# DiamondLightSource/fast-feedback-service

Measured on AMD Instinct MI355X. Metric: detector frames/s (Eiger-16M 4362x4148 uint16), higher is better.
Workload: dtype u16; 1 GPU; eiger16m: 4148x4362 uint16, 7x7 dispersion window, 32 frames/step/GPU resident in HBM, spots+centroids returned to host; streams=4, parallelism=single GPU, spot_gather=none (single GPU)

## Files before the change

fast-feedback-service_amd/csrc/ffs_context.hip:

```cpp
#include <sys/mman.h>

#include "ffs_internal.hpp"
#include "kernels_mask.hpp"

static_assert(sizeof(ReflOut) == sizeof(ffs_reflection), "record layout");
static_assert(offsetof(ReflOut, sum_intensity) == offsetof(ffs_reflection, sum_intensity), "record layout");

thread_local std::string g_create_error;

static void ctx_destroy_internal(ffs_ctx* c);
namespace {
struct Registry {
    std::mutex mu;
    std::unordered_set<const void*> live[3];
    std::atomic<bool> exiting{false};
    bool exit_hook_installed = false;
};
Registry& registry() {
    static Registry* r = new Registry();
    return *r;
}
static void on_process_exit() {
    Registry& r = registry();
    std::vector<ffs_ctx*> ctxs;
// ... 248 lines not shown
    }
    for (ffs_stream* s : streams)
        if (handle_take(kHandleStream, s)) stream_destroy_internal(s);
    for (ffs_stack3d* st : stacks)
        if (handle_take(kHandleStack, st)) {
            g_live_stacks.fetch_sub(1);
            stack3d_free(st);
        }
    ctx_destroy_internal(c);
}

static void ctx_destroy_internal(ffs_ctx* c) {
    (void)hipSetDevice(c->device);
    ahead_stop(c, true);
    for (auto* st : c->stack_pool) stack3d_free(st);
    c->stack_pool.clear();
    if (AssemblyPool* pool = c->assembly.exchange(nullptr)) {
        pool->owner.lock();
        pool->owner.unlock();
        delete pool;
    }
    if (c->d_maskbits) (void)hipFree(c->d_maskbits);
    if (c->d_gain_map) (void)hipFree(c->d_gain_map);
    if (c->d_radial_map) (void)hipFree(c->d_radial_map);
    if (c->stats_st) {
        (void)hipStreamSynchronize(c->stats_st);
        (void)hipStreamDestroy(c->stats_st);
    }
    if (c->d_stats) (void)hipFree(c->d_stats);
    if (c->d_ginfo) (void)hipFree(c->d_ginfo);
    if (c->d_mmap) (void)hipFree(c->d_mmap);
    if (c->dense_st) (void)hipStreamDestroy(c->dense_st);
    if (c->dense_st2) (void)hipStreamDestroy(c->dense_st2);
    if (c->d_handoff) (void)hipFree(c->d_handoff);
    if (c->up_st) (void)hipStreamDestroy(c->up_st);
    for (auto st : c->sparse_st) if (st) (void)hipStreamDestroy(st);
    for (auto e : c->chain_ev) if (e) (void)hipEventDestroy(e);
    for (auto& pb : c->pinned_pool) pinned_free(pb);
    delete c;
}

static int rebuild_mask_tables(ffs_ctx* c) {
    const Layout& L = c->L;
    const uint32_t gpitch = ginfo_pitch(L, c->pixel_bytes);
    HIP_TRY(c, hipMemset(c->d_ginfo, 0, (size_t)(L.H + kInfoExtraRows) * gpitch));
    const int groups = L.pitch_px / (c->pixel_bytes == 2 ? 8 : 4);
    (void)hipGetLastError();
    if (c->pixel_bytes == 2)
        hipLaunchKernelGGL(k_build_maps, dim3((groups + 255) / 256, L.H), dim3(256), 0, 0, c->d_maskbits, L.mpitch, L.W, L.H,
                           L.pitch_px, c->d_mmap, c->d_ginfo, gpitch);
    else
        hipLaunchKernelGGL(k_build_maps4, dim3((groups + 255) / 256, L.H), dim3(256), 0, 0, c->d_maskbits, L.mpitch, L.W, L.H,
                           L.pitch_px, c->d_mmap, c->d_ginfo, gpitch);
    HIP_TRY(c, hipGetLastError());
    c->empty_runs = EmptyRuns{};
    uint8_t* d_flags = nullptr;
    HIP_TRY(c, hipMalloc(reinterpret_cast<void**>(&d_flags), (size_t)L.H));
    hipLaunchKernelGGL(k_row_flags, dim3((unsigned)L.H), dim3(64), 0, 0, c->d_maskbits, L.mpitch, L.H, d_flags);
    std::vector<uint8_t> flags((size_t)L.H, 1);
    hipError_t e = hipGetLastError();
    if (e == hipSuccess) e = hipMemcpy(flags.data(), d_flags, flags.size(), hipMemcpyDeviceToHost);
    (void)hipFree(d_flags);
    HIP_TRY(c, e);
    HIP_TRY(c, hipDeviceSynchronize());
    c->empty_runs = empty_runs_of(flags.data(), L.H);
    return FFS_OK;
}

static int ffs_ctx_set_mask_impl(ffs_ctx* c, const uint8_t* host_mask) {
    if (!c) return FFS_ERR_INVALID;
    const Layout& L = c->L;
    std::vector<uint8_t> bits(L.plane_frame_stride, 0);
    const int full = L.W / 8;
    for (int y = 0; y < L.H; ++y) {
        uint8_t* row = bits.data() + (size_t)y * L.mpitch;
        if (host_mask) {
            const uint8_t* m = host_mask + (size_t)y * L.W;
            for (int g = 0; g < full; ++g) {
                uint64_t v;
                std::memcpy(&v, m + 8 * g, 8);
                const uint64_t nz = (((v & 0x7F7F7F7F7F7F7F7Full) + 0x7F7F7F7F7F7F7F7Full) | v) & 0x8080808080808080ull;
                row[g] = (uint8_t)(((nz >> 7) * 0x0102040810204080ull) >> 56);
            }
            for (int x = full * 8; x < L.W; ++x)
                if (m[x]) row[x >> 3] |= (uint8_t)(1u << (x & 7));
        } else {
            std::memset(row, 0xFF, (size_t)full);
            for (int x = full * 8; x < L.W; ++x) row[x >> 3] |= (uint8_t)(1u << (x & 7));
        }
    }
    HIP_TRY(c, hipSetDevice(c->device));
    HIP_TRY(c, hipMemcpy(c->d_maskbits, bits.data(), bits.size(), hipMemcpyHostToDevice));
    return rebuild_mask_tables(c);
}

static int ffs_ctx_get_mask_impl(ffs_ctx* c, uint8_t* host_mask) {
    if (!c || !host_mask) return FFS_ERR_INVALID;
    const Layout& L = c->L;
    std::vector<uint8_t> bits(L.plane_frame_stride);
    HIP_TRY(c, hipSetDevice(c->device));
    HIP_TRY(c, hipMemcpy(bits.data(), c->d_maskbits, bits.size(), hipMemcpyDeviceToHost));
    for (int y = 0; y < L.H; ++y)
        for (int x = 0; x < L.W; ++x)
            host_mask[(size_t)y * L.W + x] = (bits[(size_t)y * L.mpitch + (x >> 3)] >> (x & 7)) & 1;
    return FFS_OK;
}
// ... 493 lines not shown
```

fast-feedback-service_amd/csrc/kernels_mask.hpp:

```cpp
#pragma once
#include "ffs_device.h"

namespace ffsamd {

__global__ __launch_bounds__(256) void k_build_maps(const uint8_t* maskbits, uint32_t mpitch, int W, int H, int pitch_px,
                                                    uint8_t* mmap, uint8_t* ginfo, uint32_t gpitch_bytes) {
    const int g = blockIdx.x * 256 + threadIdx.x;
    const int y = blockIdx.y;
    if (g * 8 >= pitch_px) return;
    uint32_t cnt[8] = {0, 0, 0, 0, 0, 0, 0, 0};
    for (int dy = -3; dy <= 3; ++dy) {
        const int yy = y + dy;
        if (yy < 0 || yy >= H) continue;
        const uint8_t* row = maskbits + (uint64_t)yy * mpitch;
        uint32_t b = (uint32_t)row[g] << 8;
        if (g > 0) b |= row[g - 1];
        if ((uint32_t)(g + 1) < mpitch) b |= (uint32_t)row[g + 1] << 16;
        for (int j = 0; j < 8; ++j) cnt[j] += __popc((b >> (j + 5)) & 0x7Fu);
    }
    const uint32_t own = maskbits[(uint64_t)y * mpitch + g];
    uint32_t mn = 255, mx = 0;
    for (int j = 0; j < 8; ++j) {
        mmap[(uint64_t)y * pitch_px + g * 8 + j] = (uint8_t)cnt[j];
        if ((own >> j) & 1u) { mn = min(mn, cnt[j]); mx = max(mx, cnt[j]); }
    }
    if (mx == 0) mn = 0;
    ginfo[(uint64_t)y * gpitch_bytes + g * 4] = (uint8_t)own;
    ginfo[(uint64_t)(y + kInfoExtraRows) * gpitch_bytes + g * 4 + 1] = (uint8_t)mn;
    ginfo[(uint64_t)(y + kInfoExtraRows) * gpitch_bytes + g * 4 + 2] = (uint8_t)mx;
    ginfo[(uint64_t)(y + kInfoExtraRows) * gpitch_bytes + g * 4 + 3] = (uint8_t)own;
}

__global__ __launch_bounds__(256) void k_build_maps4(const uint8_t* maskbits, uint32_t mpitch, int W, int H, int pitch_px,
                                                     uint8_t* mmap, uint8_t* ginfo, uint32_t gpitch_bytes) {
    const int g = blockIdx.x * 256 + threadIdx.x;
    const int y = blockIdx.y;
    if (g * 4 >= pitch_px) return;
    uint32_t cnt[4] = {0, 0, 0, 0};
    const int byte0 = (g * 4) >> 3, sh = (g * 4) & 7;
    for (int dy = -3; dy <= 3; ++dy) {
        const int yy = y + dy;
        if (yy < 0 || yy >= H) continue;
        const uint8_t* row = maskbits + (uint64_t)yy * mpitch;
        uint32_t b = (uint32_t)row[byte0] << 8;
        if (byte0 > 0) b |= row[byte0 - 1];
        if ((uint32_t)(byte0 + 1) < mpitch) b |= (uint32_t)row[byte0 + 1] << 16;
        for (int j = 0; j < 4; ++j) cnt[j] += __popc((b >> (5 + sh + j)) & 0x7Fu);
    }
    const uint32_t own = (maskbits[(uint64_t)y * mpitch + byte0] >> sh) & 0xFu;
    uint32_t mn = 255, mx = 0;
    for (int j = 0; j < 4; ++j) {
        mmap[(uint64_t)y * pitch_px + g * 4 + j] = (uint8_t)cnt[j];
        if ((own >> j) & 1u) { mn = min(mn, cnt[j]); mx = max(mx, cnt[j]); }
    }
    if (mx == 0) mn = 0;
    ginfo[(uint64_t)y * gpitch_bytes + g * 4] = (uint8_t)own;
    ginfo[(uint64_t)(y + kInfoExtraRows) * gpitch_bytes + g * 4 + 1] = (uint8_t)mn;
    ginfo[(uint64_t)(y + kInfoExtraRows) * gpitch_bytes + g * 4 + 2] = (uint8_t)mx;
    ginfo[(uint64_t)(y + kInfoExtraRows) * gpitch_bytes + g * 4 + 3] = (uint8_t)own;
}

__global__ __launch_bounds__(64) void k_row_flags(const uint8_t* maskbits, uint32_t mpitch, int H, uint8_t* flags) {
    const int y = blockIdx.x;
    if (y >= H) return;
    const uint32_t* row = reinterpret_cast<const uint32_t*>(maskbits + (uint64_t)y * mpitch);
    uint32_t any = 0;
    for (uint32_t w = threadIdx.x; w < mpitch / 4; w += 64) any |= row[w];
    const unsigned long long m = __ballot(any != 0u);
    if (threadIdx.x == 0) flags[y] = m != 0ull ? 1 : 0;
}

__global__ void k_resolution_mask(uint8_t* maskbits, uint32_t mpitch, int W, int H, float wavelength,
                                  float distance, float cx, float cy, float psx, float psy,
                                  float dmin, float dmax) {
    const int bx = blockIdx.x * blockDim.x + threadIdx.x;
    const int y = blockIdx.y;
    if (bx * 8 >= W || y >= H) return;
    uint8_t* p = maskbits + (uint64_t)y * mpitch + bx;
    uint32_t b = *p;
    for (int j = 0; j < 8; ++j) {
        const int x = bx * 8 + j;
        if (x >= W || !((b >> j) & 1u)) continue;
        const float dx = (((float)x + 0.5f) - cx) * psx;
        const float dy = (((float)y + 0.5f) - cy) * psy;
        const float r = sqrtf(dx * dx + dy * dy);
        const float theta = 0.5f * atanf(r / distance);
        const float res = wavelength / (2.0f * sinf(theta));
        if ((dmin > 0 && res < dmin) || (dmax > 0 && res > dmax)) b &= ~(1u << j);
    }
    *p = (uint8_t)b;
}

}
```

fast-feedback-service_amd/csrc/kernels_stream.hpp:

```cpp
#pragma once
#include "kernels_threshold.hpp"

#ifndef FFS_IMG_LOAD_AUX
#define FFS_IMG_LOAD_AUX 0
#endif

namespace ffsamd {

constexpr int kSQWords = 32;

__device__ __forceinline__ bool exact_predicate(const ThresholdArgs& a, uint32_t m, unsigned long long sx,
                                                unsigned long long sy, uint32_t pc) {
    const double src = (double)pc;
    if (!((int)m >= a.min_count && src > a.threshold)) return false;
    if (a.max_valid >= 0 && (long long)pc > a.max_valid) return false;
    const double md = (double)m, xd = (double)sx, yd = (double)sy;
    const double t0 = md * yd;
    const double t1 = xd * xd;
    const double t2 = xd * (md - 1.0);
    const double av = (t0 - t1) - t2;
    const double bv = md * src - xd;
    const double cv = (xd * a.nsig_b) * __builtin_sqrt(2.0 * (md - 1.0));
    const double dv = a.nsig_s * __builtin_sqrt(xd * md);
    return av > cv && bv > dv;
// ... 71 lines not shown
__global__ __launch_bounds__(64, 4) void k_stream_u16(const ThresholdArgs a) {
    __shared__ uint32_t s_q[kSQWords][kQCap];
    __shared__ uint16_t s_list[kQCap * 8];

    const int lane = threadIdx.x;
    if (a.dbg_prio & 1) __builtin_amdgcn_s_setprio(3);
    int strip, band;
    const bool real = stream_unit(a, blockIdx.x, strip, band);
    if constexpr (!EXT)
        if (a.handoff && blockIdx.x == gridDim.x - 1 && blockIdx.y == gridDim.y - 1 && lane == 0)
            __hip_atomic_store(a.handoff, a.handoff_seq, __ATOMIC_RELEASE, __HIP_MEMORY_SCOPE_SYSTEM);
    if (!real) return;
    [[maybe_unused]] const uint32_t slot = log_slot(a, blockIdx.y, (uint32_t)band, (uint32_t)strip);
    const int f0 = blockIdx.y * a.group_frames;
    const int nf = min(a.group_frames, a.n_frames - f0);
    const int band0 = band_first_row(band, a.band_rows, a.band_rows2, a.band_split);
    const int band1 = min(band_first_row(band + 1, a.band_rows, a.band_rows2, a.band_split), a.H);
    const BandRows rows = DENSE ? BandRows{band0, band1} : trim_band(a.empty_runs, band0, band1);
    const int yb0 = rows.yb0, yb1 = rows.yb1;

    const int gsep = a.gpf + 1;
    const int G = strip * kSOwned + lane - 1;
    const int fl = G >= 0 ? G / gsep : 0;
    const int g = G - fl * gsep;
    const bool active = G >= 0 && fl < nf && g < a.gpf && yb0 != yb1;
    const bool owned = active && lane >= 1 && lane <= kSOwned;
    const uint32_t my_fg = ((uint32_t)fl << 16) | (uint32_t)g;

    const rsrc_t r_img = make_rsrc((const uint8_t*)a.image + (uint64_t)f0 * a.frame_stride,
                                   (uint32_t)((uint64_t)(nf - 1) * a.frame_stride + (uint64_t)a.H * a.pitch));
    const rsrc_t r_info = make_rsrc(a.ginfo, (uint32_t)(a.H + kInfoExtraRows) * a.gpitch);
    const rsrc_t r_sb = make_rsrc(a.strong_bytes + (uint64_t)f0 * a.bytes_frame_stride,
                                  (uint32_t)((uint64_t)nf * a.bytes_frame_stride));
    const rsrc_t r_cb = make_rsrc((EXT ? a.dplane : a.bits) + (uint64_t)f0 * a.plane_frame_stride, (uint32_t)((uint64_t)nf * a.plane_frame_stride));
    constexpr uint32_t kOob = 0x80000000u;
    const uint32_t off_px = active ? (uint32_t)((uint64_t)fl * a.frame_stride) + (uint32_t)g * 16u : kOob;
    const uint32_t off_info = active ? (uint32_t)g * 4u : kOob;
    uint32_t off_byte_st;
    {
        const uint32_t lpf = a.bpitch >> 7;
        const uint32_t u = (uint32_t)strip * 4u + ((uint32_t)lane >> 4);
        const uint32_t fz = u / lpf, cz = u - fz * lpf;
        off_byte_st = fz < (uint32_t)nf ? (uint32_t)((uint64_t)fz * a.bytes_frame_stride) + cz * 128u + ((uint32_t)lane & 15u) * 8u : kOob;
    }

    const int total = (yb1 - yb0) + (FFS_DBG(a, 1024) ? 0 : 6);
    const float kS = a.kS;

    constexpr int NS = 7 + KAHEAD;
    uint32_t ring[NS][4];
    uint32_t rinfo[NS];
    uint32_t col[8], colq[8];
    uint32_t M[4] = {0, 0, 0, 0};
    uint32_t mprev = 0;
    typedef float f32x2 __attribute__((ext_vector_type(2)));
    [[maybe_unused]] f32x2 ext_c1 = {0.0f, 0.0f}, ext_c2 = {0.0f, 0.0f};
#pragma unroll
    for (int s = 0; s < NS; ++s) {
        rinfo[s] = 0;
#pragma unroll
        for (int q = 0; q < 4; ++q) ring[s][q] = 0;
    }
#pragma unroll
    for (int j = 0; j < 8; ++j) { col[j] = 0; colq[j] = 0; }
    const unsigned long long owned_mask = __builtin_amdgcn_ballot_w64(owned);

    auto fetch = [&](int slot, int i) {
        const int yin = yb0 - 3 + i;
        const uint32_t prow = (uint32_t)min(max(yin, 0), a.H - 1);
        const uint32_t irow = (uint32_t)min(max(yin, 0), a.H + kInfoExtraRows - 1);
        const u32x4 v = __builtin_amdgcn_raw_buffer_load_b128(r_img, off_px, prow * a.pitch, FFS_IMG_LOAD_AUX);
        ring[slot][0] = v[0]; ring[slot][1] = v[1]; ring[slot][2] = v[2]; ring[slot][3] = v[3];
        rinfo[slot] = __builtin_amdgcn_raw_buffer_load_b32(r_info, off_info | (yin < 0 ? kOob : 0u), (FFS_DBG(a, 64) ? 8u : irow) * a.gpitch, 0);
    };

    auto mask_row = [&](int slot, int slot_before) {
        if (__ballot(rinfo[slot] != rinfo[slot_before]) != 0ull) {
            const uint32_t mb = rinfo[slot] & 0xFFu;
            if (__ballot(mb != mprev) != 0ull) {
#pragma unroll
                for (int q = 0; q < 4; ++q)
                    M[q] = ((uint32_t)__builtin_amdgcn_sbfe((int)mb, 2 * q, 1) & 0xFFFFu)
                         | ((uint32_t)__builtin_amdgcn_sbfe((int)mb, 2 * q + 1, 1) & 0xFFFF0000u);
                mprev = mb;
            }
            if constexpr (EXT) {
                const uint32_t mmin = (rinfo[slot] >> 8) & 0xFFu, mmax = (rinfo[slot] >> 16) & 0xFFu;
                const float mm1 = (float)mmin - 1.0f;
                const float c1 = (float)mmax * 1.0000019073486328125f;
                const float c2 = (mm1 + a.kB * __builtin_amdgcn_sqrtf(2.0f * mm1)) * 0.99999952316284179688f;
                ext_c1 = f32x2{c1, c1};
                ext_c2 = f32x2{c2, c2};
            }
        }
#pragma unroll
        for (int q = 0; q < 4; ++q) {
            ring[slot][q] &= M[q];
            asm("" : "+v"(ring[slot][q]));
        }
    };

    auto push = [&](int s, int so) {
#pragma unroll
        for (int q = 0; q < 4; ++q) {
            const uint32_t wn = ring[s][q], wo = ring[so][q];
            {
                const int32_t t = (int32_t)((wn & 0xFFFFu) - (wo & 0xFFFFu));
                const int32_t u = (int32_t)((wn & 0xFFFFu) + (wo & 0xFFFFu));
                col[2 * q] += (uint32_t)t;
                colq[2 * q] += (uint32_t)__mul24(t, u);
            }
            {
                const int32_t t = (int32_t)((wn >> 16) - (wo >> 16));
                const int32_t u = (int32_t)((wn >> 16) + (wo >> 16));
                col[2 * q + 1] += (uint32_t)t;
                colq[2 * q + 1] += (uint32_t)__mul24(t, u);
            }
        }
    };

    int qn = 0;
    [[maybe_unused]] uint32_t nlog = 0;
    [[maybe_unused]] uint32_t nbuf = 0;
    [[maybe_unused]] uint32_t lbuf[6] = {0, 0, 0, 0, 0, 0};
    [[maybe_unused]] auto flush_log = [&]() {
        const uint32_t at = nlog + (uint32_t)lane;
        if ((uint32_t)lane < nbuf && at < (uint32_t)kWlogCap && !FFS_DBG(a, 512)) {
            a.wlog[(uint64_t)slot * kWlogCap + at] = make_uint2(lbuf[0], lbuf[1]);
            a.wpix[(uint64_t)slot * kWlogCap + at] = make_uint4(lbuf[2], lbuf[3], lbuf[4], lbuf[5]);
        }
        nlog += nbuf;
        nbuf = 0;
    };
    auto drain = [&]() {
        const bool have = lane < qn && !FFS_DBG(a, 2) && !FFS_DBG(a, 32);
        uint32_t todo = 0, row = 0, fe = 0, ge = 0;
        if (have) {
            uint32_t xs[8], pws[4];
#pragma unroll
            for (int j = 0; j < 8; ++j) xs[j] = s_q[j][lane];
#pragma unroll
            for (int q = 0; q < 4; ++q) pws[q] = s_q[8 + q][lane];
            row = s_q[30][lane] >> 6;
            const uint32_t fg = s_q[31][lane];
            fe = fg >> 16;
            ge = fg & 0xFFFFu;
            const uint32_t ginf = s_q[15][lane];
            const uint32_t gmin = (ginf >> 8) & 0xFFu, gmax = (ginf >> 16) & 0xFFu;
            uint2 mm = make_uint2(gmin * 0x01010101u, gmin * 0x01010101u);
            if (gmin != gmax) {
                uint2 t = *reinterpret_cast<const uint2*>(a.mmap + (uint64_t)min(row, (uint32_t)a.H - 1u) * a.pitch_px + min(ge * 8u, (uint32_t)a.pitch_px - 8u));
                asm volatile("" : "+v"(t.x), "+v"(t.y));
                mm = t;
            }
            s_q[12][lane] = mm.x;
            s_q[13][lane] = mm.y;
            s_q[14][lane] = 0u;
            uint32_t sure = 0;
            if constexpr (EXT) {
                const uint32_t valid = ginf >> 24;
                const float kq_group = a.kB * __builtin_amdgcn_sqrtf(2.0f * ((float)gmin - 1.0f));
#pragma unroll
                for (int j = 0; j < 8; ++j) {
                    const uint32_t x = xs[j];
                    const uint32_t pw = pws[j >> 1];
                    const uint32_t pv = (j & 1) ? pw >> 16 : pw & 0xFFFFu;
                    const uint32_t m = ((j < 4 ? mm.x : mm.y) >> (8 * (j & 3))) & 0xFFu;
                    const float mf = (float)m, xf = (float)x, yf = (float)s_q[16 + j][lane];
                    const float kq = gmin == gmax ? kq_group : a.kB * __builtin_amdgcn_sqrtf(2.0f * (mf - 1.0f));
                    const float t0 = mf * yf;
                    const float af = t0 - xf * (xf + (mf - 1.0f));
                    const float cf = xf * kq;
                    const float slack = t0 * 9.5367431640625e-07f;
                    const bool bright = x >= 65536u;
                    const bool maybe = (af + slack >= cf) || bright;
                    const bool yes = !bright && (af - slack > cf * 1.000003814697265625f);
                    const bool ok = ((valid >> j) & 1u) && (int)m >= a.min_count && !(a.max_valid >= 0 && (long long)pv > a.max_valid);
                    todo |= (ok && maybe && !yes) ? (1u << j) : 0u;
                    sure |= (ok && yes) ? (1u << j) : 0u;
                }
                s_q[14][lane] = sure;
            } else {
#pragma unroll
                for (int j = 0; j < 8; ++j) {
                    const uint32_t x = xs[j];
                    const uint32_t pw = pws[j >> 1];
                    const uint32_t pv = (j & 1) ? pw >> 16 : pw & 0xFFFFu;
                    const uint32_t m = ((j < 4 ? mm.x : mm.y) >> (8 * (j & 3))) & 0xFFu;
                    const int32_t b = (int32_t)__umul24(m, pv) - (int32_t)x;
                    const float bf = (float)b, tf = (float)__umul24(x, m);
                    todo |= (bf * __builtin_fabsf(bf) > kS * tf) ? (1u << j) : 0u;
                }
            }
            if (FFS_DBG(a, 4)) todo = 0;
        }
        const uint32_t todo_n = (uint32_t)__popc(todo);
        const uint32_t todo_incl = wave_inclusive_scan(todo_n);
        const int T = __builtin_amdgcn_readlane((int)todo_incl, 63);
        {
            uint32_t pos = todo_incl - todo_n, w = todo;
            while (w) {
                const uint32_t j = (uint32_t)__ffs((int)w) - 1u;
                w &= w - 1u;
                s_list[pos++] = (uint16_t)(((uint32_t)lane << 3) | j);
            }
        }
        __builtin_amdgcn_wave_barrier();
        for (int base = 0; base < T; base += 64) {
            const int idx = base + lane;
            if (idx < T) {
                const uint32_t ent = s_list[idx], e = ent >> 3, j = ent & 7u;
                const uint32_t x = s_q[j][e], pv = (s_q[8 + (j >> 1)][e] >> (16 * (j & 1))) & 0xFFFFu;
                const uint32_t m = (s_q[12 + (j >> 2)][e] >> (8 * (j & 3))) & 0xFFu;
                uint32_t y = 0;
                if constexpr (EXT) {
                    y = s_q[16 + j][e];
                } else {
#pragma unroll
                    for (uint32_t t = 0; t < 7; ++t) y += s_q[16 + j + t][e];
                }
                asm volatile("" : "+v"(y));
                if (x < 65536u) {
                    bool certain;
                    bool strong;
                    if constexpr (EXT) {
                        strong = dispersion_only_nosqrt(a, m, x, y, certain);
                        if (!certain) strong = dispersion_only(a, m, x, y);
                    } else {
                        if (a.int_pred) strong = int_predicate(a, m, x, y, pv, certain);
                        else strong = exact_predicate_nosqrt(a, m, x, y, pv, certain);
                        if (!certain) strong = exact_predicate(a, m, x, y, pv);
                    }
                    if (strong) atomicOr(&s_q[14][e], 1u << j);
                } else if (!EXT && a.bright_to_plane) {
                    atomicOr(&s_q[14][e], 1u << j);
                } else if (!EXT && a.wlog) {
                    atomicOr(&s_q[14][e], 0x100u << j);
                } else {
                    const uint32_t tg = s_q[30][e], fgc = s_q[31][e];
                    const uint32_t fc = fgc >> 16, gc = fgc & 0xFFFFu;
                    const uint32_t at = atomicAdd(a.bright_n, 1u);
                    if (at < a.bright_cap)
                        a.bright_list[at] = make_uint2(((uint32_t)(f0 + (int)fc) << 16) | (gc * 8u + j), tg >> 6);
                }
            }
        }
        __builtin_amdgcn_wave_barrier();
        if constexpr (!EXT) if (a.wlog) {
            const uint32_t cbm = have ? s_q[14][lane] : 0u;
            const uint32_t pxw[4] = {s_q[8][lane], s_q[9][lane], s_q[10][lane], s_q[11][lane]};
            const unsigned long long wm = __builtin_amdgcn_ballot_w64(cbm != 0u);
            if (wm) {
                const uint32_t cnt = (uint32_t)__popcll(wm);
                if (nbuf + cnt > 64u) flush_log();
                const uint32_t rank = __builtin_amdgcn_mbcnt_hi((uint32_t)(wm >> 32), __builtin_amdgcn_mbcnt_lo((uint32_t)wm, 0u));
                const uint32_t dump = nbuf + cnt < 64u ? nbuf + cnt : 0u;
                const int to = (int)((cbm != 0u ? nbuf + rank : dump) << 2);
                const uint32_t e0 = (uint32_t)__builtin_amdgcn_ds_permute(to, (int)((row << 16) | ge));
                const uint32_t e1 = (uint32_t)__builtin_amdgcn_ds_permute(to, (int)((fe << 16) | cbm));
                const uint32_t p0 = (uint32_t)__builtin_amdgcn_ds_permute(to, (int)pxw[0]), p1 = (uint32_t)__builtin_amdgcn_ds_permute(to, (int)pxw[1]);
                const uint32_t p2 = (uint32_t)__builtin_amdgcn_ds_permute(to, (int)pxw[2]), p3 = (uint32_t)__builtin_amdgcn_ds_permute(to, (int)pxw[3]);
                if ((uint32_t)lane - nbuf < cnt) {
                    lbuf[0] = e0; lbuf[1] = e1;
                    lbuf[2] = p0; lbuf[3] = p1; lbuf[4] = p2; lbuf[5] = p3;
                }
                nbuf += cnt;
            }
            qn = 0;
            return;
        }
        if (have) {
            const uint32_t cb = s_q[14][lane];
            if (cb) {
                if (!FFS_DBG(a, 256)) __builtin_amdgcn_raw_buffer_store_b8((uint8_t)cb, r_cb, (uint32_t)((uint64_t)fe * a.plane_frame_stride) + ge, row * a.mpitch, 0);
                if constexpr (!EXT) if (!FFS_DBG(a, 128)) {
                    atomicAdd(a.tile_counts + (uint64_t)(f0 + (int)fe) * a.n_tiles + (row / (uint32_t)kTileRows), (uint32_t)__popc(cb));
                    const uint32_t ob = row * a.occ_spr + (ge >> 4);
                    atomicOr(a.occ + (uint64_t)(f0 + (int)fe) * a.occ_frame_words + (ob >> 5), 1u << (ob & 31u));
                }
            }
        }
        qn = 0;
    };

#pragma unroll
    for (int s = 0; s < KAHEAD; ++s) fetch(s, s);

#pragma unroll
    for (int s = 0; s < 6; ++s) {
        mask_row(s, (s + NS - 1) % NS);
        push(s, (s + KAHEAD) % NS);
        fetch((s + KAHEAD) % NS, s + KAHEAD);
    }

    for (int base = 6;; base += NS) {
#pragma unroll
        for (int t = 0; t < NS; ++t) {
            const int s = (6 + t) % NS;
            const int so = (s + KAHEAD) % NS;
            const int sc = (s + NS - 3) % NS;
            const int i = base + t;
            if (i >= total) goto rows_done;
            {
                const uint32_t info = rinfo[s];
                mask_row(s, (s + NS - 1) % NS);
                push(s, so);
                fetch(so, i + KAHEAD);

                const uint32_t s01 = col[0] + col[1], s23 = col[2] + col[3], s45 = col[4] + col[5], s67 = col[6] + col[7];
                const uint32_t ua = s01 + s23, va = s45 + s67;
                const uint32_t T0 = dpp_shr_add(s67, ua);
                const uint32_t T1 = ua + s45;
                const uint32_t T2 = va + s23;
                const uint32_t T3 = dpp_shl_add(s01, va);
                uint32_t Wn[8];
                Wn[0] = dpp_shr_add(col[5], T0);
                Wn[1] = T0 + col[4];
                Wn[2] = dpp_shr_add(col[7], T1);
                Wn[3] = T1 + col[6];
                Wn[4] = T2 + col[1];
                Wn[5] = dpp_shl_add(col[0], T2);
                Wn[6] = T3 + col[3];
                Wn[7] = dpp_shl_add(col[2], T3);

                const int yout = __builtin_amdgcn_readfirstlane(yb0 + (i - 6));
                const uint32_t so_bytes = (uint32_t)yout * a.bpitch;

                const uint32_t xmin = min(min(min(min(Wn[0], Wn[1]), Wn[2]), min(min(Wn[3], Wn[4]), Wn[5])), min(Wn[6], Wn[7]));
                const uint32_t mmin = (info >> 8) & 0xFFu, mmax = (info >> 16) & 0xFFu;
                bool pass;
                [[maybe_unused]] uint32_t ys[8];
                if constexpr (EXT) {
                    const uint32_t q01 = colq[0] + colq[1], q23 = colq[2] + colq[3], q45 = colq[4] + colq[5], q67 = colq[6] + colq[7];
                    const uint32_t qa = q01 + q23, qb = q45 + q67;
                    const uint32_t U0 = dpp_shr_add(q67, qa), U1 = qa + q45, U2 = qb + q23, U3 = dpp_shl_add(q01, qb);
                    const uint32_t y0 = dpp_shr_add(colq[5], U0), y1 = U0 + colq[4], y2 = dpp_shr_add(colq[7], U1), y3 = U1 + colq[6];
                    const uint32_t y4 = U2 + colq[1], y5 = dpp_shl_add(colq[0], U2), y6 = U3 + colq[3], y7 = dpp_shl_add(colq[2], U3);
                    ys[0] = y0; ys[1] = y1; ys[2] = y2; ys[3] = y3; ys[4] = y4; ys[5] = y5; ys[6] = y6; ys[7] = y7;
                    float dmax = -1.0f;
#pragma unroll
                    for (int jp = 0; jp < 4; ++jp) {
                        const f32x2 xf = {(float)Wn[2 * jp], (float)Wn[2 * jp + 1]};
                        const f32x2 yf = {(float)ys[2 * jp], (float)ys[2 * jp + 1]};
                        const f32x2 u = xf * (xf + ext_c2);
                        const f32x2 d = __builtin_elementwise_fma(ext_c1, yf, -u);
                        dmax = __builtin_fmaxf(dmax, __builtin_fmaxf(d.x, d.y));
                    }
                    const uint32_t xmax = max(max(max(max(Wn[0], Wn[1]), Wn[2]), max(max(Wn[3], Wn[4]), Wn[5])), max(Wn[6], Wn[7]));
                    pass = mmax != 0u && (dmax >= 0.0f || xmax >= 65536u);
                } else {
                    uint32_t pmax;
                    {
                        typedef uint16_t u16x2 __attribute__((ext_vector_type(2)));
                        const u16x2 a01 = __builtin_bit_cast(u16x2, ring[sc][0]), a23 = __builtin_bit_cast(u16x2, ring[sc][1]);
                        const u16x2 a45 = __builtin_bit_cast(u16x2, ring[sc][2]), a67 = __builtin_bit_cast(u16x2, ring[sc][3]);
                        const u16x2 mx = __builtin_elementwise_max(__builtin_elementwise_max(a01, a23), __builtin_elementwise_max(a45, a67));
                        const uint32_t mw = __builtin_bit_cast(uint32_t, mx);
                        pmax = max(mw & 0xFFFFu, mw >> 16);
                    }
                    const int32_t B = (int32_t)__umul24(mmax, pmax) - (int32_t)xmin;
                    const float bf = (float)B, tf = (float)__umul24(xmin, mmin);
                    float lhs = bf * __builtin_fabsf(bf);
                    asm("" : "+v"(lhs));
                    pass = lhs > kS * tf;
                }
                if constexpr (DENSE) __builtin_amdgcn_raw_buffer_store_b64(u32x2{0u, 0u}, r_sb, off_byte_st, so_bytes, 2 );
                const unsigned long long fm = FFS_DBG(a, 1) ? 0ull : (__builtin_amdgcn_ballot_w64(pass) & owned_mask);
                const bool flag = pass && owned;
                if (fm) {
                    const int nfl = __popcll(fm);
                    if (qn + nfl > kQCap) drain();
                    if constexpr (EXT) {
                        if (flag && !FFS_DBG(a, 32)) {
                            const uint32_t rank = __builtin_amdgcn_mbcnt_hi((uint32_t)(fm >> 32), __builtin_amdgcn_mbcnt_lo((uint32_t)fm, 0u));
                            const int e = qn + (int)rank;
#pragma unroll
                            for (int w = 0; w < 8; ++w) {
                                s_q[w][e] = Wn[w];
                                s_q[16 + w][e] = ys[w];
                            }
#pragma unroll
                            for (int w = 0; w < 4; ++w) s_q[8 + w][e] = ring[sc][w];
                            s_q[15][e] = info;
                            s_q[30][e] = ((uint32_t)yout << 6) | (uint32_t)lane; s_q[31][e] = my_fg;
                        }
                    } else {
                    const uint32_t QL5 = from_left(colq[5]), QL6 = from_left(colq[6]), QL7 = from_left(colq[7]);
                    const uint32_t QR0 = from_right(colq[0]), QR1 = from_right(colq[1]), QR2 = from_right(colq[2]);
                    if (flag && !FFS_DBG(a, 32)) {
                        const uint32_t rank = __builtin_amdgcn_mbcnt_hi((uint32_t)(fm >> 32), __builtin_amdgcn_mbcnt_lo((uint32_t)fm, 0u));
                        const int e = qn + (int)rank;
#pragma unroll
                        for (int w = 0; w < 8; ++w) {
                            s_q[w][e] = Wn[w];
                            s_q[19 + w][e] = colq[w];
                        }
#pragma unroll
                        for (int w = 0; w < 4; ++w) s_q[8 + w][e] = ring[sc][w];
                        s_q[15][e] = info;
                        s_q[16][e] = QL5; s_q[17][e] = QL6; s_q[18][e] = QL7;
                        s_q[27][e] = QR0; s_q[28][e] = QR1; s_q[29][e] = QR2;
                        s_q[30][e] = ((uint32_t)yout << 6) | (uint32_t)lane; s_q[31][e] = my_fg;
                    }
                    }
                    qn += nfl;
                }
            }
        }
    }
rows_done:
    if (qn > 0) drain();
    if constexpr (!EXT) if (a.wlog) {
        flush_log();
        if (lane == 0) a.wlog_n[slot] = FFS_DBG(a, 512) ? 0u : nlog;
    }
}
template <typename PixelT, bool EXT = false>
__global__ __launch_bounds__(256) void k_bright_fix(const ThresholdArgs a) {
    if (blockIdx.x == 0 && threadIdx.x == 0 && *a.bright_n > a.bright_cap) atomicOr(a.overflow, kOvfBrightList);
    const uint32_t n = min(*a.bright_n, a.bright_cap);
    for (uint32_t e = blockIdx.x * 256 + threadIdx.x; e < n; e += gridDim.x * 256) {
        const uint2 r = a.bright_list[e];
        const uint32_t frame = r.x >> 16, x = r.x & 0xFFFFu, y = r.y;
        const uint8_t* img = (const uint8_t*)a.image + (uint64_t)frame * a.frame_stride;
        if (exact_strong<PixelT, EXT>(a, img, (int)x, (int)y)) {
            uint8_t* plane = (EXT ? a.dplane : a.bits) + (uint64_t)frame * a.plane_frame_stride + (uint64_t)y * a.mpitch;
            atomicOr(reinterpret_cast<uint32_t*>(plane) + (x >> 5), 1u << (x & 31u));
            if (!EXT) {
                atomicAdd(a.tile_counts + (uint64_t)frame * a.n_tiles + y / (uint32_t)kTileRows, 1u);
                const uint32_t ob = y * a.occ_spr + (x >> 7);
                atomicOr(a.occ + (uint64_t)frame * a.occ_frame_words + (ob >> 5), 1u << (ob & 31u));
            }
        }
    }
}


constexpr int kS4Words = 32;

template <int KAHEAD, bool DENSE = false>
__global__ __launch_bounds__(64, 4) void k_stream_u32(const ThresholdArgs a) {
    __shared__ uint32_t s_q[kS4Words][kQCap];
    __shared__ uint16_t s_list[kQCap * 4];

    const int lane = threadIdx.x;
    int strip, band;
    const bool real = stream_unit(a, blockIdx.x, strip, band);
    if (a.handoff && blockIdx.x == gridDim.x - 1 && blockIdx.y == gridDim.y - 1 && lane == 0)
        __hip_atomic_store(a.handoff, a.handoff_seq, __ATOMIC_RELEASE, __HIP_MEMORY_SCOPE_SYSTEM);
    if (!real) return;
    const uint32_t slot = log_slot(a, blockIdx.y, (uint32_t)band, (uint32_t)strip);
    const int f0 = blockIdx.y * a.group_frames;
    const int nf = min(a.group_frames, a.n_frames - f0);
    const int band0 = band_first_row(band, a.band_rows, a.band_rows2, a.band_split);
    const int band1 = min(band_first_row(band + 1, a.band_rows, a.band_rows2, a.band_split), a.H);
    const BandRows rows = DENSE ? BandRows{band0, band1} : trim_band(a.empty_runs, band0, band1);
    const int yb0 = rows.yb0, yb1 = rows.yb1;

    const int gsep = a.gpf + 1;
    const int G = strip * kSOwned + lane - 1;
    const int fl = G >= 0 ? G / gsep : 0;
    const int g = G - fl * gsep;
    const bool active = G >= 0 && fl < nf && g < a.gpf && yb0 != yb1;
    const bool owned = active && lane >= 1 && lane <= kSOwned;

    const rsrc_t r_img = make_rsrc((const uint8_t*)a.image + (uint64_t)f0 * a.frame_stride,
                                   (uint32_t)((uint64_t)(nf - 1) * a.frame_stride + (uint64_t)a.H * a.pitch));
    const rsrc_t r_info = make_rsrc(a.ginfo, (uint32_t)(a.H + kInfoExtraRows) * a.gpitch);
    const rsrc_t r_sb = make_rsrc(a.strong_bytes + (uint64_t)f0 * a.bytes_frame_stride,
                                  (uint32_t)((uint64_t)nf * a.bytes_frame_stride));
    constexpr uint32_t kOob = 0x80000000u;
    const uint32_t off_px = active ? (uint32_t)((uint64_t)fl * a.frame_stride) + (uint32_t)g * 16u : kOob;
    const uint32_t off_info = active ? (uint32_t)g * 4u : kOob;
    uint32_t off_byte_st;
    {
        const uint32_t lpf = a.bpitch >> 7;
        const uint32_t u = (uint32_t)strip * 2u + ((uint32_t)lane >> 4);
        const uint32_t fz = u / lpf, cz = u - fz * lpf;
        off_byte_st = (lane < 32 && fz < (uint32_t)nf) ? (uint32_t)((uint64_t)fz * a.bytes_frame_stride) + cz * 128u + ((uint32_t)lane & 15u) * 8u : kOob;
    }

    const int total = (yb1 - yb0) + 6;
    const float kS = a.kS;

    constexpr int NS = 7 + KAHEAD;
    uint32_t ring[NS][4];
    uint32_t rinfo[NS];
    uint32_t col[4];
    long long colq[4];
    uint32_t M[4] = {0, 0, 0, 0};
    uint32_t mprev = 0;
    uint32_t bighist = 0;
#pragma unroll
    for (int s = 0; s < NS; ++s) {
        rinfo[s] = 0;
#pragma unroll
        for (int q = 0; q < 4; ++q) ring[s][q] = 0;
    }
#pragma unroll
    for (int j = 0; j < 4; ++j) { col[j] = 0; colq[j] = 0; }
    const unsigned long long owned_mask = __builtin_amdgcn_ballot_w64(owned);

    auto fetch = [&](int slot, int i) {
        const int yin = yb0 - 3 + i;
        const uint32_t prow = (uint32_t)min(max(yin, 0), a.H - 1);
        const uint32_t irow = (uint32_t)min(max(yin, 0), a.H + kInfoExtraRows - 1);
        const u32x4 v = __builtin_amdgcn_raw_buffer_load_b128(r_img, off_px, prow * a.pitch, FFS_IMG_LOAD_AUX);
        ring[slot][0] = v[0]; ring[slot][1] = v[1]; ring[slot][2] = v[2]; ring[slot][3] = v[3];
        rinfo[slot] = __builtin_amdgcn_raw_buffer_load_b32(r_info, off_info | (yin < 0 ? kOob : 0u), irow * a.gpitch, 0);
    };

    auto mask_row = [&](int slot, int slot_before) {
        if (__ballot(rinfo[slot] != rinfo[slot_before]) != 0ull) {
            const uint32_t mb = rinfo[slot] & 0xFu;
            if (__ballot(mb != mprev) != 0ull) {
#pragma unroll
                for (int q = 0; q < 4; ++q) M[q] = (uint32_t)__builtin_amdgcn_sbfe((int)mb, q, 1);
                mprev = mb;
            }
        }
#pragma unroll
        for (int q = 0; q < 4; ++q) ring[slot][q] &= M[q];
    };

    auto push = [&](int s, int so) {
        const uint32_t big = ((ring[s][0] | ring[s][1]) | (ring[s][2] | ring[s][3])) >> 24 ? 1u : 0u;
        bighist = (bighist & ~((1u << s) | (1u << so))) | (big << s);
#pragma unroll
        for (int q = 0; q < 4; ++q) {
            const int32_t t = (int32_t)(ring[s][q] - ring[so][q]), u = (int32_t)(ring[s][q] + ring[so][q]);
            col[q] += (uint32_t)t;
            colq[q] += (long long)t * (long long)u;
        }
    };

    int qn = 0;
    uint32_t nlog = 0;
    uint32_t nbuf = 0;
    uint32_t lbuf[6] = {0, 0, 0, 0, 0, 0};
    auto flush_log = [&]() {
        const uint32_t at = nlog + (uint32_t)lane;
        if ((uint32_t)lane < nbuf && at < (uint32_t)kWlogCap) {
            a.wlog[(uint64_t)slot * kWlogCap + at] = make_uint2(lbuf[0], lbuf[1]);
            a.wpix[(uint64_t)slot * kWlogCap + at] = make_uint4(lbuf[2], lbuf[3], lbuf[4], lbuf[5]);
        }
        nlog += nbuf;
        nbuf = 0;
    };
    auto drain = [&]() {
        const bool have = lane < qn && !FFS_DBG(a, 2) && !FFS_DBG(a, 32);
        uint32_t todo = 0, row = 0, fe = 0, ge = 0, info = 0;
        bool big = false;
        if (have) {
            const uint32_t tag = s_q[11][lane], ln = tag & 63u;
            big = (tag >> 31) != 0u;
            row = (tag & 0x7FFFFFFFu) >> 6;
            const int Ge = strip * kSOwned + (int)ln - 1;
            fe = (uint32_t)Ge / (uint32_t)gsep;
            ge = (uint32_t)Ge - fe * (uint32_t)gsep;
            info = s_q[8][lane];
            uint32_t xs[4], pvs[4];
#pragma unroll
            for (int j = 0; j < 4; ++j) { xs[j] = s_q[j][lane]; pvs[j] = s_q[4 + j][lane]; }
            const uint32_t gmin = (info >> 8) & 0xFFu, gmax = (info >> 16) & 0xFFu;
            uint32_t mm = gmin * 0x01010101u;
            if (gmin != gmax) {
                uint32_t t = *reinterpret_cast<const uint32_t*>(a.mmap + (uint64_t)min(row, (uint32_t)a.H - 1u) * a.pitch_px
                                                                + min(ge * 4u, (uint32_t)a.pitch_px - 4u));
                asm volatile("" : "+v"(t));
                mm = t;
            }
            s_q[9][lane] = mm;
            s_q[10][lane] = 0u;
            if (!big) {
#pragma unroll
                for (int j = 0; j < 4; ++j) {
                    const uint32_t x = xs[j], pv = pvs[j];
                    const uint32_t m = (mm >> (8 * j)) & 0xFFu;
                    const int32_t b = (int32_t)(m * pv) - (int32_t)x;
                    const float bf = (float)b, tf = (float)x * (float)m;
                    todo |= (bf * __builtin_fabsf(bf) > kS * tf) ? (1u << j) : 0u;
                }
            }
        }
        if (__ballot(big) != 0ull) {
            if (big && a.bright_to_plane) {
                s_q[10][lane] = (info >> 24) & 0xFu;
            } else if (big && a.wlog) {
                s_q[10][lane] = ((info >> 24) & 0xFu) << 8;
            } else if (big) {
                for (uint32_t j = 0; j < 4; ++j) {
                    if (!((info >> (24 + j)) & 1u)) continue;
                    const uint32_t at = atomicAdd(a.bright_n, 1u);
                    if (at < a.bright_cap) a.bright_list[at] = make_uint2(((uint32_t)(f0 + (int)fe) << 16) | (ge * 4u + j), row);
                }
            }
        }
        const uint32_t todo_n = (uint32_t)__popc(todo);
        const uint32_t todo_incl = wave_inclusive_scan(todo_n);
        const int T = __builtin_amdgcn_readlane((int)todo_incl, 63);
        {
            uint32_t pos = todo_incl - todo_n, w = todo;
            while (w) {
                const uint32_t j = (uint32_t)__ffs((int)w) - 1u;
                w &= w - 1u;
                s_list[pos++] = (uint16_t)(((uint32_t)lane << 2) | j);
            }
        }
        __builtin_amdgcn_wave_barrier();
        for (int base = 0; base < T; base += 64) {
            const int idx = base + lane;
            if (idx < T) {
                const uint32_t ent = s_list[idx], e = ent >> 2, j = ent & 3u;
                const uint32_t x = s_q[j][e], pv = s_q[4 + j][e];
                const uint32_t m = (s_q[9][e] >> (8 * j)) & 0xFFu;
                unsigned long long y = 0;
#pragma unroll
                for (uint32_t t = 0; t < 7; ++t)
                    y += ((unsigned long long)s_q[22 + j + t][e] << 32) | s_q[12 + j + t][e];
                bool certain = false, strong = false;
                if (y < (1ull << 46)) strong = exact_predicate_nosqrt(a, m, x, y, pv, certain);
                if (!certain) strong = exact_predicate(a, m, x, y, pv);
                if (strong) atomicOr(&s_q[10][e], 1u << j);
            }
        }
        __builtin_amdgcn_wave_barrier();
        if (a.wlog) {
            const uint32_t cbm = have ? s_q[10][lane] : 0u;
            const uint32_t pxw[4] = {s_q[4][lane], s_q[5][lane], s_q[6][lane], s_q[7][lane]};
            const unsigned long long wm = __builtin_amdgcn_ballot_w64(cbm != 0u);
            if (wm) {
                const uint32_t cnt = (uint32_t)__popcll(wm);
                if (nbuf + cnt > 64u) flush_log();
                const uint32_t rank = __builtin_amdgcn_mbcnt_hi((uint32_t)(wm >> 32), __builtin_amdgcn_mbcnt_lo((uint32_t)wm, 0u));
                const uint32_t dump = nbuf + cnt < 64u ? nbuf + cnt : 0u;
                const int to = (int)((cbm != 0u ? nbuf + rank : dump) << 2);
                const uint32_t e0 = (uint32_t)__builtin_amdgcn_ds_permute(to, (int)((row << 16) | ge));
                const uint32_t e1 = (uint32_t)__builtin_amdgcn_ds_permute(to, (int)((fe << 16) | cbm));
                const uint32_t p0 = (uint32_t)__builtin_amdgcn_ds_permute(to, (int)pxw[0]), p1 = (uint32_t)__builtin_amdgcn_ds_permute(to, (int)pxw[1]);
                const uint32_t p2 = (uint32_t)__builtin_amdgcn_ds_permute(to, (int)pxw[2]), p3 = (uint32_t)__builtin_amdgcn_ds_permute(to, (int)pxw[3]);
                if ((uint32_t)lane - nbuf < cnt) {
                    lbuf[0] = e0; lbuf[1] = e1;
                    lbuf[2] = p0; lbuf[3] = p1; lbuf[4] = p2; lbuf[5] = p3;
                }
                nbuf += cnt;
            }
            qn = 0;
            return;
        }
        if (have) {
            const uint32_t cb = s_q[10][lane];
            if (cb) {
                const uint32_t x0 = ge * 4u;
                uint32_t* plane = reinterpret_cast<uint32_t*>(a.bits + (uint64_t)(f0 + (int)fe) * a.plane_frame_stride + (uint64_t)row * a.mpitch);
                atomicOr(plane + (x0 >> 5), cb << (x0 & 31u));
                atomicAdd(a.tile_counts + (uint64_t)(f0 + (int)fe) * a.n_tiles + (row / (uint32_t)kTileRows), (uint32_t)__popc(cb));
                const uint32_t ob = row * a.occ_spr + (x0 >> 7);
                atomicOr(a.occ + (uint64_t)(f0 + (int)fe) * a.occ_frame_words + (ob >> 5), 1u << (ob & 31u));
            }
        }
        qn = 0;
    };

#pragma unroll
    for (int s = 0; s < KAHEAD; ++s) fetch(s, s);
#pragma unroll
    for (int s = 0; s < 6; ++s) {
        mask_row(s, (s + NS - 1) % NS);
        push(s, (s + KAHEAD) % NS);
        fetch((s + KAHEAD) % NS, s + KAHEAD);
    }

    for (int base = 6;; base += NS) {
#pragma unroll
        for (int t = 0; t < NS; ++t) {
            const int s = (6 + t) % NS;
            const int so = (s + KAHEAD) % NS;
            const int sc = (s + NS - 3) % NS;
            const int i = base + t;
            if (i >= total) goto rows_done;
            {
                const uint32_t info = rinfo[s];
                mask_row(s, (s + NS - 1) % NS);
                push(s, so);
                fetch(so, i + KAHEAD);

                const uint32_t s01 = col[0] + col[1], s23 = col[2] + col[3];
                const uint32_t S = s01 + s23;
                const uint32_t TL = dpp_shr_add(s23, S);
                const uint32_t TR = dpp_shl_add(s01, S);
                uint32_t Wn[4];
                Wn[0] = dpp_shr_add(col[1], TL);
                Wn[1] = dpp_shl_add(col[0], TL);
                Wn[2] = dpp_shr_add(col[3], TR);
                Wn[3] = dpp_shl_add(col[2], TR);

                const int yout = __builtin_amdgcn_readfirstlane(yb0 + (i - 6));
                if constexpr (DENSE) __builtin_amdgcn_raw_buffer_store_b64(u32x2{0u, 0u}, r_sb, off_byte_st, (uint32_t)yout * a.bpitch, 2);

                const uint32_t xmin = min(min(min(Wn[0], Wn[1]), Wn[2]), Wn[3]);
                const uint32_t pmax = max(max(max(ring[sc][0], ring[sc][1]), ring[sc][2]), ring[sc][3]);
                const uint32_t mmin = (info >> 8) & 0xFFu, mmax = (info >> 16) & 0xFFu;
                const int32_t B = (int32_t)(mmax * pmax) - (int32_t)xmin;
                const float bf = (float)B, tf = (float)xmin * (float)mmin;
                const bool pass = bf * __builtin_fabsf(bf) > kS * tf;
                const uint32_t bl = bighist != 0u ? 1u : 0u;
                bool near_big = false;
                if (__ballot(bl != 0u) != 0ull) near_big = (bl | from_left(bl) | from_right(bl)) != 0u && mmax != 0u;
                const bool want = pass || near_big;
                const unsigned long long fm = FFS_DBG(a, 1) ? 0ull : (__builtin_amdgcn_ballot_w64(want) & owned_mask);
                const bool flag = want && owned;
                if (fm) {
                    const int nfl = __popcll(fm);
                    if (qn + nfl > kQCap) drain();
                    uint32_t ql[4], qh[4];
#pragma unroll
                    for (int w = 0; w < 4; ++w) { ql[w] = (uint32_t)colq[w]; qh[w] = (uint32_t)((unsigned long long)colq[w] >> 32); }
                    const uint32_t QL1 = from_left(ql[1]), QL2 = from_left(ql[2]), QL3 = from_left(ql[3]);
                    const uint32_t QR0 = from_right(ql[0]), QR1 = from_right(ql[1]), QR2 = from_right(ql[2]);
                    const uint32_t HL1 = from_left(qh[1]), HL2 = from_left(qh[2]), HL3 = from_left(qh[3]);
                    const uint32_t HR0 = from_right(qh[0]), HR1 = from_right(qh[1]), HR2 = from_right(qh[2]);
                    if (flag && !FFS_DBG(a, 32)) {
                        const uint32_t rank = __builtin_amdgcn_mbcnt_hi((uint32_t)(fm >> 32), __builtin_amdgcn_mbcnt_lo((uint32_t)fm, 0u));
                        const int e = qn + (int)rank;
#pragma unroll
                        for (int w = 0; w < 4; ++w) {
                            s_q[w][e] = Wn[w];
                            s_q[4 + w][e] = ring[sc][w];
                            s_q[15 + w][e] = ql[w];
                            s_q[25 + w][e] = qh[w];
                        }
                        s_q[8][e] = info;
                        s_q[12][e] = QL1; s_q[13][e] = QL2; s_q[14][e] = QL3;
                        s_q[19][e] = QR0; s_q[20][e] = QR1; s_q[21][e] = QR2;
                        s_q[22][e] = HL1; s_q[23][e] = HL2; s_q[24][e] = HL3;
                        s_q[29][e] = HR0; s_q[30][e] = HR1; s_q[31][e] = HR2;
                        s_q[11][e] = ((uint32_t)yout << 6) | (uint32_t)lane | (near_big ? 0x80000000u : 0u);
                    }
                    qn += nfl;
                }
            }
        }
    }
rows_done:
    if (qn > 0) drain();
    if (a.wlog) {
        flush_log();
        if (lane == 0) a.wlog_n[slot] = nlog;
    }
}

template __global__ void k_bright_fix<uint16_t>(const ThresholdArgs);
template __global__ void k_bright_fix<uint16_t, true>(const ThresholdArgs);
template __global__ void k_bright_fix<uint32_t>(const ThresholdArgs);

template __global__ void k_stream_u16<2, false, false>(const ThresholdArgs);
template __global__ void k_stream_u16<3, false, false>(const ThresholdArgs);
template __global__ void k_stream_u16<4, false, false>(const ThresholdArgs);
template __global__ void k_stream_u16<2, false, true>(const ThresholdArgs);
template __global__ void k_stream_u16<2, true, false>(const ThresholdArgs);
template __global__ void k_stream_u16<2, true, true>(const ThresholdArgs);
template __global__ void k_stream_u32<2, false>(const ThresholdArgs);
template __global__ void k_stream_u32<3, false>(const ThresholdArgs);
template __global__ void k_stream_u32<2, true>(const ThresholdArgs);

}
```

Measured before the change: 119,100 frames/s.

## Load per-pixel mask counts during row streaming instead of in drain

Moves the per-pixel mask-count (mmap) load out of the candidate drain path and into mask_row, where it runs only when the row's ginfo word changes, then carries the counts through the shared queue slots. A new setup kernel decrements a ginfo byte wherever the count vector changes between rows while the info word is unchanged, so the row-change ballot fires exactly when the counts must be reloaded. This removes scattered global loads from the drain phase but adds register pressure and queue stores in the hot loop. It also changes slot usage in the shared queue (slot 15 is no longer written on one path), which risks subtle correctness issues.

```diff
diff --git a/fast-feedback-service_amd/csrc/ffs_context.hip b/fast-feedback-service_amd/csrc/ffs_context.hip
--- a/fast-feedback-service_amd/csrc/ffs_context.hip
+++ b/fast-feedback-service_amd/csrc/ffs_context.hip
@@ -324,6 +324,11 @@
     else
         hipLaunchKernelGGL(k_build_maps4, dim3((groups + 255) / 256, L.H), dim3(256), 0, 0, c->d_maskbits, L.mpitch, L.W, L.H,
                            L.pitch_px, c->d_mmap, c->d_ginfo, gpitch);
+    HIP_TRY(c, hipGetLastError());
+    if (c->pixel_bytes == 2)
+        hipLaunchKernelGGL(k_mark_count_changes<8>, dim3((groups + 63) / 64), dim3(64), 0, 0, c->d_mmap, L.H, L.pitch_px, c->d_ginfo, gpitch);
+    else
+        hipLaunchKernelGGL(k_mark_count_changes<4>, dim3((groups + 63) / 64), dim3(64), 0, 0, c->d_mmap, L.H, L.pitch_px, c->d_ginfo, gpitch);
     HIP_TRY(c, hipGetLastError());
     c->empty_runs = EmptyRuns{};
     uint8_t* d_flags = nullptr;
diff --git a/fast-feedback-service_amd/csrc/kernels_mask.hpp b/fast-feedback-service_amd/csrc/kernels_mask.hpp
--- a/fast-feedback-service_amd/csrc/kernels_mask.hpp
+++ b/fast-feedback-service_amd/csrc/kernels_mask.hpp
@@ -60,6 +60,27 @@
     ginfo[(uint64_t)(y + kInfoExtraRows) * gpitch_bytes + g * 4 + 3] = (uint8_t)own;
 }
 
+template <int PX>
+__global__ __launch_bounds__(64) void k_mark_count_changes(const uint8_t* mmap, int H, int pitch_px, uint8_t* ginfo, uint32_t gpitch_bytes) {
+    const int g = blockIdx.x * 64 + threadIdx.x;
+    if (g * PX >= pitch_px) return;
+    uint32_t p0 = 0, p1 = 0;
+    uint32_t dp = *reinterpret_cast<const uint32_t*>(ginfo + (uint64_t)(kInfoExtraRows - 1) * gpitch_bytes + g * 4);
+#pragma unroll 4
+    for (int y = 0; y < H; ++y) {
+        const uint8_t* at = mmap + (uint64_t)y * pitch_px + g * PX;
+        const uint32_t c0 = *reinterpret_cast<const uint32_t*>(at);
+        const uint32_t c1 = PX == 8 ? *reinterpret_cast<const uint32_t*>(at + 4) : 0u;
+        uint32_t* dw = reinterpret_cast<uint32_t*>(ginfo + (uint64_t)(y + kInfoExtraRows) * gpitch_bytes + g * 4);
+        uint32_t d = *dw;
+        if ((c0 != p0 || c1 != p1) && d == dp && (d & 0xFF0000u) != 0u) {
+            d -= 0x100u;
+            *dw = d;
+        }
+        p0 = c0; p1 = c1; dp = d;
+    }
+}
+
 __global__ __launch_bounds__(64) void k_row_flags(const uint8_t* maskbits, uint32_t mpitch, int H, uint8_t* flags) {
     const int y = blockIdx.x;
     if (y >= H) return;
diff --git a/fast-feedback-service_amd/csrc/kernels_stream.hpp b/fast-feedback-service_amd/csrc/kernels_stream.hpp
--- a/fast-feedback-service_amd/csrc/kernels_stream.hpp
+++ b/fast-feedback-service_amd/csrc/kernels_stream.hpp
@@ -147,7 +147,8 @@
     uint32_t rinfo[NS];
     uint32_t col[8], colq[8];
     uint32_t M[4] = {0, 0, 0, 0};
-    uint32_t mprev = 0;
+    [[maybe_unused]] uint32_t mprev = 0;
+    uint2 mm = make_uint2(0u, 0u);
     typedef float f32x2 __attribute__((ext_vector_type(2)));
     [[maybe_unused]] f32x2 ext_c1 = {0.0f, 0.0f}, ext_c2 = {0.0f, 0.0f};
 #pragma unroll
@@ -169,15 +170,28 @@
         rinfo[slot] = __builtin_amdgcn_raw_buffer_load_b32(r_info, off_info | (yin < 0 ? kOob : 0u), (FFS_DBG(a, 64) ? 8u : irow) * a.gpitch, 0);
     };
 
-    auto mask_row = [&](int slot, int slot_before) {
+    auto mask_row = [&](int slot, int slot_before, int yc) {
         if (__ballot(rinfo[slot] != rinfo[slot_before]) != 0ull) {
             const uint32_t mb = rinfo[slot] & 0xFFu;
-            if (__ballot(mb != mprev) != 0ull) {
+            uint32_t mb_before;
+            if constexpr (EXT) mb_before = rinfo[slot_before] & 0xFFu; else mb_before = mprev;
+            if (__ballot(mb != mb_before) != 0ull) {
 #pragma unroll
                 for (int q = 0; q < 4; ++q)
                     M[q] = ((uint32_t)__builtin_amdgcn_sbfe((int)mb, 2 * q, 1) & 0xFFFFu)
                          | ((uint32_t)__builtin_amdgcn_sbfe((int)mb, 2 * q + 1, 1) & 0xFFFF0000u);
                 mprev = mb;
+            }
+            {
+                uint32_t ri = rinfo[slot];
+                asm("" : "+v"(ri));
+                const uint32_t cmin = (ri >> 8) & 0xFFu, cmax = (ri >> 16) & 0xFFu;
+                uint2 t = make_uint2(cmin * 0x01010101u, cmin * 0x01010101u);
+                if (cmin != cmax) {
+                    t = *reinterpret_cast<const uint2*>(a.mmap + (uint64_t)(uint32_t)min(max(yc, 0), a.H - 1) * a.pitch_px + (uint32_t)g * 8u);
+                    asm volatile("" : "+v"(t.x), "+v"(t.y));
+                }
+                mm = t;
             }
             if constexpr (EXT) {
                 const uint32_t mmin = (rinfo[slot] >> 8) & 0xFFu, mmax = (rinfo[slot] >> 16) & 0xFFu;
@@ -240,19 +254,12 @@
             const uint32_t fg = s_q[31][lane];
             fe = fg >> 16;
             ge = fg & 0xFFFFu;
-            const uint32_t ginf = s_q[15][lane];
-            const uint32_t gmin = (ginf >> 8) & 0xFFu, gmax = (ginf >> 16) & 0xFFu;
-            uint2 mm = make_uint2(gmin * 0x01010101u, gmin * 0x01010101u);
-            if (gmin != gmax) {
-                uint2 t = *reinterpret_cast<const uint2*>(a.mmap + (uint64_t)min(row, (uint32_t)a.H - 1u) * a.pitch_px + min(ge * 8u, (uint32_t)a.pitch_px - 8u));
-                asm volatile("" : "+v"(t.x), "+v"(t.y));
-                mm = t;
-            }
-            s_q[12][lane] = mm.x;
-            s_q[13][lane] = mm.y;
+            const uint2 qm = make_uint2(s_q[12][lane], s_q[13][lane]);
             s_q[14][lane] = 0u;
             uint32_t sure = 0;
             if constexpr (EXT) {
+                const uint32_t ginf = s_q[15][lane];
+                const uint32_t gmin = (ginf >> 8) & 0xFFu, gmax = (ginf >> 16) & 0xFFu;
                 const uint32_t valid = ginf >> 24;
                 const float kq_group = a.kB * __builtin_amdgcn_sqrtf(2.0f * ((float)gmin - 1.0f));
 #pragma unroll
@@ -260,7 +267,7 @@
                     const uint32_t x = xs[j];
                     const uint32_t pw = pws[j >> 1];
                     const uint32_t pv = (j & 1) ? pw >> 16 : pw & 0xFFFFu;
-                    const uint32_t m = ((j < 4 ? mm.x : mm.y) >> (8 * (j & 3))) & 0xFFu;
+                    const uint32_t m = ((j < 4 ? qm.x : qm.y) >> (8 * (j & 3))) & 0xFFu;
                     const float mf = (float)m, xf = (float)x, yf = (float)s_q[16 + j][lane];
                     const float kq = gmin == gmax ? kq_group : a.kB * __builtin_amdgcn_sqrtf(2.0f * (mf - 1.0f));
                     const float t0 = mf * yf;
@@ -281,7 +288,7 @@
                     const uint32_t x = xs[j];
                     const uint32_t pw = pws[j >> 1];
                     const uint32_t pv = (j & 1) ? pw >> 16 : pw & 0xFFFFu;
-                    const uint32_t m = ((j < 4 ? mm.x : mm.y) >> (8 * (j & 3))) & 0xFFu;
+                    const uint32_t m = ((j < 4 ? qm.x : qm.y) >> (8 * (j & 3))) & 0xFFu;
                     const int32_t b = (int32_t)__umul24(m, pv) - (int32_t)x;
                     const float bf = (float)b, tf = (float)__umul24(x, m);
                     todo |= (bf * __builtin_fabsf(bf) > kS * tf) ? (1u << j) : 0u;
@@ -383,7 +390,7 @@
 
 #pragma unroll
     for (int s = 0; s < 6; ++s) {
-        mask_row(s, (s + NS - 1) % NS);
+        mask_row(s, (s + NS - 1) % NS, yb0 + s - 6);
         push(s, (s + KAHEAD) % NS);
         fetch((s + KAHEAD) % NS, s + KAHEAD);
     }
@@ -398,7 +405,7 @@
             if (i >= total) goto rows_done;
             {
                 const uint32_t info = rinfo[s];
-                mask_row(s, (s + NS - 1) % NS);
+                mask_row(s, (s + NS - 1) % NS, yb0 + (i - 6));
                 push(s, so);
                 fetch(so, i + KAHEAD);
 
@@ -476,6 +483,7 @@
                             }
 #pragma unroll
                             for (int w = 0; w < 4; ++w) s_q[8 + w][e] = ring[sc][w];
+                            s_q[12][e] = mm.x; s_q[13][e] = mm.y;
                             s_q[15][e] = info;
                             s_q[30][e] = ((uint32_t)yout << 6) | (uint32_t)lane; s_q[31][e] = my_fg;
                         }
@@ -492,7 +500,7 @@
                         }
 #pragma unroll
                         for (int w = 0; w < 4; ++w) s_q[8 + w][e] = ring[sc][w];
-                        s_q[15][e] = info;
+                        s_q[12][e] = mm.x; s_q[13][e] = mm.y;
                         s_q[16][e] = QL5; s_q[17][e] = QL6; s_q[18][e] = QL7;
                         s_q[27][e] = QR0; s_q[28][e] = QR1; s_q[29][e] = QR2;
                         s_q[30][e] = ((uint32_t)yout << 6) | (uint32_t)lane; s_q[31][e] = my_fg;
@@ -585,6 +593,7 @@
     long long colq[4];
     uint32_t M[4] = {0, 0, 0, 0};
     uint32_t mprev = 0;
+    uint32_t mm = 0;
     uint32_t bighist = 0;
 #pragma unroll
     for (int s = 0; s < NS; ++s) {
@@ -605,7 +614,7 @@
         rinfo[slot] = __builtin_amdgcn_raw_buffer_load_b32(r_info, off_info | (yin < 0 ? kOob : 0u), irow * a.gpitch, 0);
     };
 
-    auto mask_row = [&](int slot, int slot_before) {
+    auto mask_row = [&](int slot, int slot_before, int yc) {
         if (__ballot(rinfo[slot] != rinfo[slot_before]) != 0ull) {
             const uint32_t mb = rinfo[slot] & 0xFu;
             if (__ballot(mb != mprev) != 0ull) {
@@ -613,6 +622,15 @@
                 for (int q = 0; q < 4; ++q) M[q] = (uint32_t)__builtin_amdgcn_sbfe((int)mb, q, 1);
                 mprev = mb;
             }
+            uint32_t ri = rinfo[slot];
+            asm("" : "+v"(ri));
+            const uint32_t cmin = (ri >> 8) & 0xFFu, cmax = (ri >> 16) & 0xFFu;
+            uint32_t t = cmin * 0x01010101u;
+            if (cmin != cmax) {
+                t = *reinterpret_cast<const uint32_t*>(a.mmap + (uint64_t)(uint32_t)min(max(yc, 0), a.H - 1) * a.pitch_px + (uint32_t)g * 4u);
+                asm volatile("" : "+v"(t));
+            }
+            mm = t;
         }
 #pragma unroll
         for (int q = 0; q < 4; ++q) ring[slot][q] &= M[q];
@@ -657,21 +675,13 @@
             uint32_t xs[4], pvs[4];
 #pragma unroll
             for (int j = 0; j < 4; ++j) { xs[j] = s_q[j][lane]; pvs[j] = s_q[4 + j][lane]; }
-            const uint32_t gmin = (info >> 8) & 0xFFu, gmax = (info >> 16) & 0xFFu;
-            uint32_t mm = gmin * 0x01010101u;
-            if (gmin != gmax) {
-                uint32_t t = *reinterpret_cast<const uint32_t*>(a.mmap + (uint64_t)min(row, (uint32_t)a.H - 1u) * a.pitch_px
-                                                                + min(ge * 4u, (uint32_t)a.pitch_px - 4u));
-                asm volatile("" : "+v"(t));
-                mm = t;
-            }
-            s_q[9][lane] = mm;
+            const uint32_t qm = s_q[9][lane];
             s_q[10][lane] = 0u;
             if (!big) {
 #pragma unroll
                 for (int j = 0; j < 4; ++j) {
                     const uint32_t x = xs[j], pv = pvs[j];
-                    const uint32_t m = (mm >> (8 * j)) & 0xFFu;
+                    const uint32_t m = (qm >> (8 * j)) & 0xFFu;
                     const int32_t b = (int32_t)(m * pv) - (int32_t)x;
                     const float bf = (float)b, tf = (float)x * (float)m;
                     todo |= (bf * __builtin_fabsf(bf) > kS * tf) ? (1u << j) : 0u;
@@ -761,7 +771,7 @@
     for (int s = 0; s < KAHEAD; ++s) fetch(s, s);
 #pragma unroll
     for (int s = 0; s < 6; ++s) {
-        mask_row(s, (s + NS - 1) % NS);
+        mask_row(s, (s + NS - 1) % NS, yb0 + s - 6);
         push(s, (s + KAHEAD) % NS);
         fetch((s + KAHEAD) % NS, s + KAHEAD);
     }
@@ -776,7 +786,7 @@
             if (i >= total) goto rows_done;
             {
                 const uint32_t info = rinfo[s];
-                mask_row(s, (s + NS - 1) % NS);
+                mask_row(s, (s + NS - 1) % NS, yb0 + (i - 6));
                 push(s, so);
                 fetch(so, i + KAHEAD);
 
@@ -826,6 +836,7 @@
                             s_q[25 + w][e] = qh[w];
                         }
                         s_q[8][e] = info;
+                        s_q[9][e] = mm;
                         s_q[12][e] = QL1; s_q[13][e] = QL2; s_q[14][e] = QL3;
                         s_q[19][e] = QR0; s_q[20][e] = QR1; s_q[21][e] = QR2;
                         s_q[22][e] = HL1; s_q[23][e] = HL2; s_q[24][e] = HL3;
```

Result: no change. 120,000 frames/s, median of 2 (+0.7%).
